# SamvitJ/Accel

Hardware: AMD Instinct MI355X
Metric: frames/sec 1024x2048 Accel-18 kf=5 (higher is better)
Workload: dtype f32 (storage, accumulation and results; the launch geometries the tuner picks include the fp32 MFMA, Winograd F(2x2,3x3) and, for most layers, 'fp16x2': each fp32 operand as TWO half terms hi + lo (22-23 significant bits, operands centred in the half range by exact powers of two: weights per channel

## Files before the change

### accel_amd/csrc/accel_hip.cpp

```cpp
#include <hip/hip_runtime.h>
#include <dlfcn.h>
#include <sys/stat.h>
#include <unistd.h>

#include <algorithm>
#include <cmath>
#include <cstdarg>
#include <cstdio>
#include <cstdlib>
#include <cstring>
#include <map>
#include <memory>
#include <sstream>
#include <string>
#include <vector>

#include "../../include/accel_hip.h"
#include "kernels.h"
#include "range.h"

static thread_local std::string g_err;

static int fail(int code, const char* fmt, ...)
{
// ... 474 lines not shown
        c.yH = op.b.H; c.yW = op.b.W;
        if (op.b.H > 2 * op.a.H || op.b.H < 2 * op.a.H - 1 || op.b.W > 2 * op.a.W || op.b.W < 2 * op.a.W - 1)
            return fail(ACCEL_ERR_PLAN, "deconv2x %s: output must be 2x the input (or one row / column less)", op.name.c_str());
    } else {
        int wkh = kh, wkw = kw;
        if (cols) kv_pair(kv, "wk", wkh, wkw, 3, 3);
        if (w->shape[0] != cout || w->shape[1] != cin || w->shape[2] != wkh || w->shape[3] != wkw)
            return fail(ACCEL_ERR_PARAM, "shape inconsistent for %s: need (%d,%d,%d,%d) got (%ld,%ld,%ld,%ld)",
                        wname.c_str(), cout, cin, wkh, wkw, (long)w->shape[0], (long)w->shape[1], (long)w->shape[2], (long)w->shape[3]);
        const int Kreal = wkh * wkw * cin_pad;
        c.K_pad = roundup(Kreal, 32);
        pack_conv_w(*w, cin_pad, rows, c.K_pad, packed);
        if (cols) { c.kh = c.kw = 1; c.Cin = Kreal; }
        else { c.kh = kh; c.kw = kw; c.Cin = cin_pad; }
        c.sh = sh; c.sw = sw; c.ph = ph; c.pw = pw; c.dh = dh; c.dw = dw;
        c.Ho = op.b.H; c.Wo = op.b.W;
        c.yH = op.b.H; c.yW = op.b.W;
        const int eh = (op.a.H + 2 * c.ph - c.dh * (c.kh - 1) - 1) / c.sh + 1;
        const int ew = (op.a.W + 2 * c.pw - c.dw * (c.kw - 1) - 1) / c.sw + 1;
        if (eh != op.b.H || ew != op.b.W)
            return fail(ACCEL_ERR_PLAN, "conv %s: output %dx%d does not match geometry %dx%d", op.name.c_str(), op.b.H, op.b.W, eh, ew);
        if (c.Cin > op.a.Cs) return fail(ACCEL_ERR_PLAN, "conv %s: input view narrower than Cin", op.name.c_str());
    }
    packed.resize(packed.size() + 256, 0.f);
    const char* env_dt = getenv("ACCEL_CONV_DTYPE");
    const int dflt = (p->f16 == 2 || (env_dt && !strcmp(env_dt, "bf16x3"))) ? 2 : (p->f16 || (env_dt && !strcmp(env_dt, "f16"))) ? 1 : 0;
    const int want_f16 = (int)kv_int(kv, "f16", dflt);
    c.f16 = (want_f16 && c.Cin % (want_f16 == 2 ? 4 : 8) == 0 && cout_store > 4) ? want_f16 : 0;
    void* dw_ = nullptr;
    if (c.f16 == 2) {
        std::vector<uint16_t> pb;
        pack_bf16x3(packed, c.deconv2x ? 4 : 1, rows, c.K_pad, pb, c.w_plane);
        if ((rc = dev_upload(p, pb.data(), pb.size() * sizeof(uint16_t), &dw_))) return rc;
    } else if (c.f16) {
        std::vector<_Float16> ph(packed.size());
        for (size_t i = 0; i < packed.size(); ++i) ph[i] = (_Float16)packed[i];
        if ((rc = dev_upload(p, ph.data(), ph.size() * sizeof(_Float16), &dw_))) return rc;
        if (!withheld("b3r")) {
            const int classes = c.deconv2x ? 4 : 1, steps = c.K_pad / 32;
            c.w_plane = (size_t)classes * rows * c.K_pad + 2 * (size_t)rows * 32;
            std::vector<_Float16> pr(c.w_plane, (_Float16)0.f);
            for (int cl = 0; cl < classes; ++cl)
                for (int n = 0; n < rows; ++n)
                    for (int k = 0; k < c.K_pad; ++k)
                        pr[((((size_t)cl * steps + k / 32) * 2 + ((k >> 4) & 1)) * rows + n) * 16 + (k & 15)] = ph[((size_t)cl * rows + n) * c.K_pad + k];
            void* d4 = nullptr;
            if ((rc = dev_upload(p, pr.data(), pr.size() * sizeof(_Float16), &d4))) return rc;
            c.wb3r = d4;
        }
    } else if ((rc = dev_upload(p, packed.data(), packed.size() * sizeof(float), &dw_))) return rc;
    c.w = static_cast<const float*>(dw_);
    {
        const int ft = (int)kv_int(kv, "tile", -1);
        const bool forced = (ft >= CONV_TILE_B3 && ft < CONV_TILE_B3D + CONV_TILE_B3D_N) || (ft >= 90 && ft <= 96);
        if (!c.f16 && c.Cin % 4 == 0 && cout_store > 4 && (!withheld("split") || forced)) {
            std::vector<uint16_t> pb;
            pack_bf16x3(packed, c.deconv2x ? 4 : 1, rows, c.K_pad, pb, c.w_plane);
            void* d3 = nullptr;
            if ((rc = dev_upload(p, pb.data(), pb.size() * sizeof(uint16_t), &d3))) return rc;
            c.wb3 = d3;
            const bool forced_r = (ft >= CONV_TILE_B3R && ft < CONV_TILE_B3D + CONV_TILE_B3D_N) || (ft >= 90 && ft <= 96);
            if (!withheld("b3r") || forced_r) {
                pack_bf16x3r(packed, c.deconv2x ? 4 : 1, rows, c.K_pad, pb, c.w_plane);
                void* d4 = nullptr;
                if ((rc = dev_upload(p, pb.data(), pb.size() * sizeof(uint16_t), &d4))) return rc;
                c.wb3r = d4;
            }
        } else if (forced && !(c.f16 == 1 && c.wb3r && ft >= CONV_TILE_B3R && ft < CONV_TILE_B3D + CONV_TILE_B3D_N)) {
            return fail(ACCEL_ERR_ARG, "conv %s: the bf16x3 kernel takes layers with more than "
                                       "4 output channels only", op.name.c_str());
        }
    }

    std::vector<float> scale(rows, 0.f), shift(rows, 0.f);
    for (int i = 0; i < cout; ++i) scale[i] = 1.f;
    if (kv_has(kv, "bn")) {
        std::vector<float> s, b;
        if ((rc = bn_fold(m, kv_str(kv, "bn"), (float)kv_f(kv, "eps", 1e-5), (int)kv_int(kv, "fixg", 0), cout, s, b))) return rc;
        for (int i = 0; i < cout; ++i) { scale[i] = s[i]; shift[i] = b[i]; }
    }
    if (kv_has(kv, "bias")) {
        const HostParam* bias = get_param(m, kv_str(kv, "bias"));
        if (!bias) return fail(ACCEL_ERR_PARAM, "%s not initialized", kv_str(kv, "bias").c_str());
        if ((int)bias->numel() != cout) return fail(ACCEL_ERR_PARAM, "shape inconsistent for %s", kv_str(kv, "bias").c_str());
        for (int i = 0; i < cout; ++i) shift[i] += bias->data[i] * scale[i];
    }
    if (kv_has(kv, "mul")) {
        const float mul = (float)kv_f(kv, "mul", 1.0);
        for (int i = 0; i < cout; ++i) { scale[i] *= mul; shift[i] *= mul; }
    }
    void *ds = nullptr, *db = nullptr;
    if ((rc = dev_upload(p, scale.data(), rows * sizeof(float), &ds)) ||
        (rc = dev_upload(p, shift.data(), rows * sizeof(float), &db))) return rc;
    c.scale = static_cast<const float*>(ds);
    c.shift = static_cast<const float*>(db);
    {
        const char* sp = getenv("ACCEL_SPLIT");
        const bool h2 = sp ? !strcmp(sp, "h2") : p->split == 1;
        if (c.wb3r && !c.f16 && h2) {
            std::vector<uint16_t> ph;
            std::vector<int> q;
            pack_h2r(packed, c.deconv2x ? 4 : 1, rows, c.K_pad, ph, c.w_plane, q);
            void *dh = nullptr, *dsh = nullptr;
            if ((rc = dev_upload(p, ph.data(), ph.size() * sizeof(uint16_t), &dh))) return rc;
            std::vector<float> sh(rows);
            for (int i = 0; i < rows; ++i) sh[i] = std::ldexp(scale[i], -q[i]);
            if ((rc = dev_upload(p, sh.data(), rows * sizeof(float), &dsh))) return rc;
            c.wh2r = dh;
            c.scale_h2 = static_cast<const float*>(dsh);
            ++p->n_h2;
        }
    }
    if (op.c.set) {
        std::vector<float> s2(rows, 0.f), b2(rows, 0.f), s, b;
// ... 95 lines not shown
        } else if (c.force_tile == CONV_TILE_WINO || c.force_tile == CONV_TILE_WINO_B3 || c.force_tile == CONV_TILE_WINO_B3U || c.force_tile == CONV_TILE_WINO_B3S) {
            return fail(ACCEL_ERR_ARG, "conv %s: the Winograd kernel takes 3x3 / stride 1 / dilation 1 / pad 1 layers with even output "
                                       "size and channels in multiples of 8 only", op.name.c_str());
        }
    }
    {
        const bool want = !withheld("stem") || c.force_tile == CONV_TILE_STEM || c.force_tile == CONV_TILE_STEM_B3;
        c.Cout_store = cout_store;
        c.res = op.d.set ? op.d.ptr : nullptr;
        if (want && !cols && cin == 3 && cout == 64 && conv_stem_eligible(c)) {
            std::vector<float> ws((size_t)conv_stem_pack_floats(), 0.f);
            conv_stem_pack(w->data.data(), cout, ws.data());
            void* dsw = nullptr;
            if ((rc = dev_upload(p, ws.data(), ws.size() * sizeof(float), &dsw))) return rc;
            c.wstem = static_cast<const float*>(dsw);
            if ((!withheld("split") && !withheld("stem_split")) || c.force_tile == CONV_TILE_STEM_B3) {
                std::vector<unsigned short> wb;
                conv_stem_b3_pack(w->data.data(), cout, wb);
                void* dsb = nullptr;
                if ((rc = dev_upload(p, wb.data(), wb.size() * sizeof(unsigned short), &dsb))) return rc;
                c.wstemb = dsb;
                if (c.wh2r) {
                    std::vector<int> q;
                    conv_stem_b3_pack_h2(w->data.data(), cout, wb, q);
                    void *dh = nullptr, *dsh = nullptr;
                    if ((rc = dev_upload(p, wb.data(), wb.size() * sizeof(unsigned short), &dh))) return rc;
                    std::vector<float> sh(rows, 0.f);
                    for (int i = 0; i < rows && i < 64; ++i) sh[i] = std::ldexp(scale[i], -q[i]);
                    if ((rc = dev_upload(p, sh.data(), rows * sizeof(float), &dsh))) return rc;
                    c.wstemh = dh;
                    c.scale_h2s = static_cast<const float*>(dsh);
                }
            }
        } else if (c.force_tile == CONV_TILE_STEM || c.force_tile == CONV_TILE_STEM_B3) {
            return fail(ACCEL_ERR_ARG, "conv %s: the stem kernel takes 7x7 / stride 2 / pad 3 layers on 3-channel images with 64 "
                                       "output channels only", op.name.c_str());
        }
    }
    {
        const bool want = !withheld("ws1x1") || c.force_tile == CONV_TILE_WS;
        c.y2 = op.c.set ? op.c.ptr : nullptr;
        if (want && !cols && cin == cin_pad && conv_ws_eligible(c)) {
            std::vector<float> ww(conv_ws_pack_floats(cin, cout_store), 0.f);
            conv_ws_pack(w->data.data(), cout, cin, cout_store, ww.data());
            void* dw = nullptr;
            if ((rc = dev_upload(p, ww.data(), ww.size() * sizeof(float), &dw))) return rc;
            c.wws = static_cast<const float*>(dw);
            c.wws_bytes = (unsigned)(ww.size() * sizeof(float));
        } else if (c.force_tile == CONV_TILE_WS) {
            return fail(ACCEL_ERR_ARG, "conv %s: the weight-stationary kernel takes 1x1 / stride 1 layers from 64 to a multiple of 256 "
                                       "or from 128 to a multiple of 128 channels (ReLU or no activation, one output) only", op.name.c_str());
        }
    }
    c.narrow = (cout_store == 4 && !c.deconv2x && !op.c.set && c.force_tile < 0 && kv_int(kv, "narrow", 1)) ? 1 : 0;
    c.no_split = (int)kv_int(kv, "nosplit", 0);
    c.split_target = (int)kv_int(kv, "split_target", 0);
    const size_t ws = conv_plan_split(c);
    if (ws > p->ws_bytes) p->ws_bytes = ws;
    return 0;
}

static int upload_param(accel_plan* p, const std::string& name, size_t expect, const float** out)
{
    const HostParam* h = get_param(p->m, name);
    if (!h) return fail(ACCEL_ERR_PARAM, "%s not initialized", name.c_str());
    if (expect && h->numel() != expect) return fail(ACCEL_ERR_PARAM, "shape inconsistent for %s: %zu elements, expected %zu", name.c_str(), h->numel(), expect);
    void* d = nullptr;
    int rc = dev_upload(p, h->data.data(), h->numel() * sizeof(float), &d);
    if (rc) return rc;
    *out = static_cast<const float*>(d);
    return 0;
}

static int input_slot(accel_plan* p, const BufRef& r, const float* const** out)
{
    *out = nullptr;
    if (r.space == "A" || r.off != 0) return 0;
    DevBuf& b = p->m->pbufs[r.space];
    ++b.prep_readers;
    if (!b.slot) {
        void* d = nullptr;
        HIP_TRY(hipMalloc(&d, sizeof(void*)));
        b.slot = static_cast<const void**>(d);
        HIP_TRY(hipMemcpy(d, &b.ptr, sizeof(void*), hipMemcpyHostToDevice));
    }
    *out = reinterpret_cast<const float* const*>(b.slot);
    return 0;
}

static int scores_buffer(accel_plan* p, Op& op, const ScoreTailParams& q)
{
    const int zCs = roundup(q.ncls, 4);
    const size_t zbytes = (size_t)op.a.N * q.Hs * q.Ws * zCs * sizeof(float);
    DevBuf& zb = p->m->pbufs["scores"];
    if (!zb.ptr) {
        HIP_TRY(hipMalloc(&zb.ptr, zbytes));
        zb.bytes = zbytes;
        HIP_TRY(hipMemsetAsync(zb.ptr, 0, zbytes, p->m->ctx->stream));
    } else if (zb.bytes != zbytes) {
        return fail(ACCEL_ERR_PLAN, "score_tail %s: the model's `scores` buffer has %zu bytes, this plan needs %zu", op.name.c_str(), zb.bytes, zbytes);
    }
    op.tail_z = static_cast<float*>(zb.ptr);
    op.tail_lowres = q;
    op.tail_lowres.left = op.tail_z; op.tail_lowres.lCs = zCs;
    op.tail_lowres.right = nullptr; op.tail_lowres.wr = nullptr;
    op.tail_lowres.uniform_w = 1;
// ... 211 lines not shown
    const ConvParams& c = op.conv;
    hipError_t e = hipSuccess;
    if (op.measure) e = launch_range_amax(c.x, (long)op.a.N * c.H * c.W, c.Cin, c.xCs, const_cast<unsigned*>(c.xr_slot), p->m->ctx->stream);
    if (e == hipSuccess && (op.measure || op.fold)) e = launch_range_fold(const_cast<unsigned*>(c.xr_slot), p->range_flag_dev, (int)(&op - p->ops.data()), p->m->ctx->stream);
    if (e != hipSuccess) return fail(ACCEL_ERR_HIP, "range pass of conv %s failed: %s", op.name.c_str(), hipGetErrorString(e));
    return 0;
}

static int run_eager(accel_plan* p)
{
    if (p->n_slots && launch_range_clear(p->range, p->n_slots, p->m->ctx->stream) != hipSuccess)
        return fail(ACCEL_ERR_HIP, "clearing the range slots of plan '%s' failed", p->role.c_str());
    for (size_t i = 0; i < p->ops.size(); ++i) {
        Op& op = p->ops[i];
        int rc = (op.measure || op.fold) ? launch_measure(p, op) : 0;
        if (!rc) rc = launch_op(p, op);
        if (rc) return rc;
        static const char* chk = getenv("ACCEL_CHECK_FINITE");
        if (chk && chk[0] == '1' && !p->gexec && (op.kind == OP_CONV || op.kind == OP_POOL || op.kind == OP_PREP_RGB) && p->n_slots) {
            const BufRef& o = op.b;
            if (o.esize == 4 && o.ptr && p->check_scratch) {
                unsigned* scratch = p->check_scratch;
                hipStream_t st = p->m->ctx->stream;
                launch_range_clear(scratch, 1, st);
                launch_range_amax(o.ptr, (long)o.N * o.H * o.W, roundup(o.C, 4), o.Cs, scratch, st);
                launch_range_fold(scratch, nullptr, 0, st);
                unsigned bits = 0;
                hipStreamSynchronize(st);
                hipMemcpy(&bits, scratch, 4, hipMemcpyDeviceToHost);
                if (bits >= 0x7F800000u) fprintf(stderr, "[accel check] plan %s op %zu %s %s: output holds a non-finite value (largest |x| bits 0x%08x)\n", p->role.c_str(), i, op.kind_name.c_str(), op.name.c_str(), bits);
            }
        }
    }
    return 0;
}

static int range_check(accel_plan* p)
{
    if (!p->range_flag || !*p->range_flag) return 0;
    const unsigned w = *p->range_flag, i = (w & 0x7FFFFFFFu) - 1u;
    *p->range_flag = 0u;
    return fail(ACCEL_ERR_RANGE, "plan '%s': the input of conv %s was not finite in an earlier run (the largest |value| stored into it was %s; fp16x2 "
                "form of the fp32 layers: the frames of that run are not trustworthy; ACCEL_SPLIT=b3 selects the bf16x3 form, which propagates "
                "non-finite values like fp32 arithmetic)",
                p->role.c_str(), i < p->ops.size() ? p->ops[i].name.c_str() : "?", (w & 0x80000000u) ? "a NaN" : "an infinity");
}

static bool conv_has_h2_form(const ConvParams& c) { return c.wh2r || c.wubh || c.wstemh; }
static bool conv_runs_h2(const ConvParams& c)
{
    if (c.f16 || c.narrow) return false;
    const int t = c.force_tile;
    return ((t == CONV_TILE_WINO_B3 || t == CONV_TILE_WINO_B3U || t == CONV_TILE_WINO_B3S) && c.wubh) || (t == CONV_TILE_STEM_B3 && c.wstemh) ||
           (((t >= CONV_TILE_B3R && t < CONV_TILE_B3R + 6) || (t >= 90 && t <= 96)) && c.wh2r);
}

static int assign_range_slots(accel_plan* p)
{
    std::map<int, int>& slot_of = p->slot_of;
    int n = 0;
    p->in_slot.assign(p->ops.size(), -1);
    for (size_t i = 0; i < p->ops.size(); ++i) {
        Op& op = p->ops[i];
        if (op.kind != OP_CONV || !conv_has_h2_form(op.conv)) continue;
        if (op.rs_in < 0) p->in_slot[i] = n++;
        else {
            auto it = slot_of.find(op.rs_in);
            if (it == slot_of.end()) it = slot_of.insert({op.rs_in, n++}).first;
            p->in_slot[i] = it->second;
        }
    }
    p->n_slots = n;
    if (!n) return 0;
    HIP_TRY(hipMalloc((void**)&p->range, (size_t)(n + 1) * RANGE_WORDS * sizeof(unsigned)));
    p->owned.push_back(p->range);
    HIP_TRY(hipMemset(p->range, 0, (size_t)(n + 1) * RANGE_WORDS * sizeof(unsigned)));
    p->check_scratch = p->range + (size_t)n * RANGE_WORDS;
    HIP_TRY(hipHostMalloc((void**)&p->range_flag, 2 * sizeof(unsigned), hipHostMallocMapped));
    p->range_flag[0] = p->range_flag[1] = 0u;
    HIP_TRY(hipHostGetDevicePointer((void**)&p->range_flag_dev, p->range_flag, 0));
    for (size_t i = 0; i < p->ops.size(); ++i)
        if (p->in_slot[i] >= 0) p->ops[i].conv.xr_slot = p->range + (size_t)p->in_slot[i] * RANGE_WORDS;
    return 0;
}

static void resolve_range_flags(accel_plan* p, bool (*counts)(const ConvParams&))
{
    const int n = p->n_slots;
    if (!n) return;
    std::vector<char> used(n, 0);
    for (size_t i = 0; i < p->ops.size(); ++i)
        if (p->in_slot[i] >= 0 && counts(p->ops[i].conv)) used[p->in_slot[i]] = 1;
    auto addr = [&](int id) -> unsigned* {
        auto it = id < 0 ? p->slot_of.end() : p->slot_of.find(id);
        return (it == p->slot_of.end() || !used[it->second]) ? nullptr : p->range + (size_t)it->second * RANGE_WORDS;
    };
    std::vector<int> state(n, 0);
    std::vector<char> dirty(n, 0);
    auto wrote = [&](int id, bool has_epilogue) {
        auto it = id < 0 ? p->slot_of.end() : p->slot_of.find(id);
        if (it == p->slot_of.end()) return;
        int& st = state[it->second];
        st = (has_epilogue && st != 2) ? 1 : 2;
        dirty[it->second] = 1;
    };
    for (size_t i = 0; i < p->ops.size(); ++i) {
        Op& op = p->ops[i];
// ... 128 lines not shown
    const char* e = getenv("ACCEL_AUTOTUNE");
    if (e && e[0] == '0') return 0;
    hipStream_t st = p->m->ctx->stream;
    tune_cache_load();
    bool tuned_any = false;
    struct Cand { int tile, split_target, no_split; };
    std::vector<std::vector<Cand>> cands(p->ops.size());
    size_t ws_need = p->ws_bytes;
    for (size_t i = 0; i < p->ops.size(); ++i) {
        Op& op = p->ops[i];
        if (op.kind != OP_CONV || op.conv.force_tile >= 0 || op.conv.narrow) continue;
        ConvParams c = op.conv;
        std::vector<Cand>& cs = cands[i];
        if (c.x_half || c.y_half || c.res_half) {
            for (int t : {CONV_TILE_B3D, CONV_TILE_B3D + 1, CONV_TILE_B3D + 2, CONV_TILE_B3D + 3, CONV_TILE_B3D + 6, CONV_TILE_B3D + 7}) {
                if ((t == CONV_TILE_B3D || t == CONV_TILE_B3D + 1) && c.Cout_store <= 128) continue;
                if ((t != CONV_TILE_B3D + 6) && c.Cout_store <= 64) continue;
                cs.push_back({t, 0, 0});
                ConvParams q = c;
                const size_t base = conv_apply(q, t, 0, 0);
                const int ks0 = q.ksplit;
                if (conv_apply(q, t, 1024, 0) && q.ksplit != ks0) cs.push_back({t, 1024, 0});
                if (base) cs.push_back({t, 0, 1});
            }
        }
        else if (c.f16 && c.Cout_store <= 32) { cs.push_back({3, 0, 0}); cs.push_back({3, 1024, 0}); }
        else if (c.Cout_store <= 32) {
            cs.push_back({4, 0, 0}); cs.push_back({4, 1024, 0}); cs.push_back({9, 0, 0}); cs.push_back({9, 1024, 0}); cs.push_back({3, 0, 0});
            if (c.wh2r && conv_halo_eligible(c) && !withheld("halo")) cs.push_back({CONV_TILE_HALO, 0, 1});
        }
        else {
            if (c.wu && !c.f16) {
                cs.push_back({CONV_TILE_WINO, 0, 0});
                ConvParams q = c;
                const size_t base = conv_apply(q, CONV_TILE_WINO, 0, 0);
                const int ks0 = q.ksplit;
                if (conv_apply(q, CONV_TILE_WINO, 1024, 0) && q.ksplit != ks0) cs.push_back({CONV_TILE_WINO, 1024, 0});
                if (base) cs.push_back({CONV_TILE_WINO, 0, 1});
            }
            if (c.wub && !c.f16) {
                for (int wt : {CONV_TILE_WINO_B3, CONV_TILE_WINO_B3U, CONV_TILE_WINO_B3S}) {
                    cs.push_back({wt, 0, 0});
                    ConvParams q = c;
                    const size_t base = conv_apply(q, wt, 0, 0);
                    const int ks0 = q.ksplit;
                    if (conv_apply(q, wt, 1024, 0) && q.ksplit != ks0) cs.push_back({wt, 1024, 0});
                    if (base) cs.push_back({wt, 0, 1});
                }
            }
            if (c.wstem && !c.f16) cs.push_back({CONV_TILE_STEM, 0, 0});
            if (c.wstemb && !c.f16) cs.push_back({CONV_TILE_STEM_B3, 0, 0});
            if (c.wws && !c.f16) cs.push_back({CONV_TILE_WS, 0, 0});
            if (c.wh2r && !c.f16 && conv_halo_eligible(c) && !withheld("halo")) cs.push_back({CONV_TILE_HALO, 0, 1});
            const int nb3 = c.wb3 ? 5 : 0;
            static const int tiles[] = {0, 1, 2, 3, 5, 6, 7, 8, 10, 11, 12, 13, 31, 32, 33, 34, 35,
                                        CONV_TILE_B3, CONV_TILE_B3 + 1, CONV_TILE_B3 + 2, CONV_TILE_B3 + 3, CONV_TILE_B3 + 4, CONV_TILE_B3 + 5,
                                        CONV_TILE_B3R, CONV_TILE_B3R + 1, CONV_TILE_B3R + 3, CONV_TILE_B3R + 4, CONV_TILE_B3R + 5};
            const bool no_deep = withheld("deep");
            for (int t : tiles) {
                if (t >= CONV_TILE_B3 && t < CONV_TILE_B3R && !nb3) continue;
                if (t >= CONV_TILE_B3R && !c.wb3r) continue;
                if (no_deep && t >= 31 && t <= 35) continue;
                if (c.K_pad % conv_tile_bk(t)) continue;
                if (c.f16 && !(t <= 3 || t == 10 || (c.f16 == 1 && t >= CONV_TILE_B3R && c.wb3r))) continue;
                cs.push_back({t, 0, 0});
                ConvParams q = c;
                const size_t base = conv_apply(q, t, 0, 0);
                const int ks0 = q.ksplit;
                if (conv_apply(q, t, 1024, 0) && q.ksplit != ks0) cs.push_back({t, 1024, 0});
                if (base) cs.push_back({t, 0, 1});
            }
        }
        if (const char* fw = getenv("ACCEL_WB3_FORCE"); fw && c.wub && !c.f16) {
            cs.clear();
            conv_apply(op.conv, atoi(fw), 0, 0);
            ConvParams q = op.conv;
            const size_t w = conv_plan_split(q);
            if (w > ws_need) ws_need = w;
            continue;
        }
        for (const Cand& k : cs) { ConvParams q = c; size_t w = conv_apply(q, k.tile, k.split_target, k.no_split); if (w > ws_need) ws_need = w; }
    }
    if (ws_need > p->ws_bytes) {
        float* nw = nullptr;
        HIP_TRY(hipMalloc((void**)&nw, ws_need));
        poison(nw, ws_need);
        p->owned.push_back(nw);
        p->ws = nw; p->ws_bytes = ws_need;
        for (Op& op : p->ops) if (op.kind == OP_CONV) op.conv.ws = p->ws;
    }
    struct TuneScratch {
        hipEvent_t e0 = nullptr, e1 = nullptr;
        void* scrub = nullptr;
        hipStream_t st;
        ~TuneScratch()
        {
            if (e0) hipEventDestroy(e0);
            if (e1) hipEventDestroy(e1);
            if (scrub) { hipStreamSynchronize(st); hipFree(scrub); }
        }
    } ts;
    ts.st = st;
    HIP_TRY(hipEventCreate(&ts.e0)); HIP_TRY(hipEventCreate(&ts.e1));
    hipEvent_t e0 = ts.e0, e1 = ts.e1;
    int rc = 0;
    const size_t scrub_bytes = (size_t)320 << 20;
// ... 1437 lines not shown
```

### accel_amd/csrc/conv_igemm.hip

```cpp
#include <hip/hip_runtime.h>
#include <cstdlib>
#include "kernels.h"
#include "conv_common.h"

#ifdef ACCEL_CONV_TIMELINE
__device__ unsigned long long g_conv_timeline[8 * 16384];
#define CONV_TL(slot) do { if (threadIdx.x == 0 && blockIdx.y == 0 && blockIdx.z == 0 && blockIdx.x < 16384) \
        g_conv_timeline[blockIdx.x * 8 + (slot)] = __builtin_amdgcn_s_memrealtime(); } while (0)
extern "C" int accel_debug_conv_timeline(unsigned long long* out, int n)
{
    return (int)hipMemcpyFromSymbol(out, HIP_SYMBOL(g_conv_timeline), sizeof(unsigned long long) * (size_t)n);
}
#else
#define CONV_TL(slot) do { } while (0)
#endif

#include "conv_epilogue.h"

template <int BM, int BN, int WGM, int WGN, int BK, int MID, int ABL = 0, int FAST = 0>
__global__ __launch_bounds__(64 * WGM * WGN) void conv_igemm_f32_kernel(ConvParams p)
{
    constexpr int LDK = BK + 4;
    constexpr int NTHR = 64 * WGM * WGN;
    constexpr int CPR = BK / 4;
// ... 935 lines not shown
    ConvParams p = p0;
    p.MT = (p.M + BM - 1) / BM;
    p.NT = (p.Cout_store + BN - 1) / BN;
    constexpr bool WDMA = WGM * WGN == 8;
    constexpr size_t lds = WDMA ? (size_t)(3 * BM * 40 + 2 * 3 * BN * 32) * sizeof(unsigned short) : (size_t)3 * (BM + BN) * 40 * sizeof(unsigned short);
    if (hipError_t e = ensure_dynamic_lds(reinterpret_cast<const void*>(&conv_igemm_b3_kernel<BM, BN, WGM, WGN, WDMA, true>), lds); e != hipSuccess) return e;
    if (hipError_t e = ensure_dynamic_lds(reinterpret_cast<const void*>(&conv_igemm_b3_kernel<BM, BN, WGM, WGN, WDMA, false>), lds); e != hipSuccess) return e;
    dim3 grid(p.MT * p.NT, p.deconv2x ? 4 : 1, p.ksplit > 1 ? p.ksplit : 1);
    if (p.Cin % 32 == 0) hipLaunchKernelGGL((conv_igemm_b3_kernel<BM, BN, WGM, WGN, WDMA, true>), grid, dim3(64 * WGM * WGN), lds, st, p, p.w_plane);
    else hipLaunchKernelGGL((conv_igemm_b3_kernel<BM, BN, WGM, WGN, WDMA, false>), grid, dim3(64 * WGM * WGN), lds, st, p, p.w_plane);
    hipError_t e = hipGetLastError();
    if (e != hipSuccess || p.ksplit <= 1) return e;
    const long total = (long)grid.y * p.M * (p.Cout_store / 4);
    hipLaunchKernelGGL(splitk_reduce_kernel, dim3((unsigned)((total + 255) / 256)), dim3(256), 0, st, p, (int)grid.y);
    return hipGetLastError();
}

int conv_pick_tile(const ConvParams& p)
{
    if (p.force_tile >= 0) return p.force_tile;
    if (p.x_half || p.y_half || p.res_half) return p.Cout_store <= 64 ? CONV_TILE_B3D + 6 : CONV_TILE_B3D + 2;
    const long classes = p.deconv2x ? 4 : 1;
    const int cs = p.Cout_store;
    if (cs <= 32) return p.f16 ? 3 : 4;
    auto blocks = [&](int bm, int bn) {
        return classes * ((p.M + bm - 1) / bm) * (long)((cs + bn - 1) / bn);
    };
    if (cs <= 64) return blocks(128, 64) >= 512 ? 1 : 3;
    if (blocks(128, 128) < 64) return 3;
    if (cs % 128 == 0 || cs > 256) {
        if (blocks(128, 128) >= 512) return 0;
        if (blocks(128, 64) >= 512) return 1;
        if (blocks(64, 128) >= 384) return 2;
        return 3;
    }
    if (blocks(128, 64) >= 512) return 1;
    return 3;
}

hipError_t launch_splitk_reduce(const ConvParams& p, int classes, hipStream_t st)
{
    const long total = (long)classes * p.M * (p.Cout_store / 4);
    hipLaunchKernelGGL(splitk_reduce_kernel, dim3((unsigned)((total + 255) / 256)), dim3(256), 0, st, p, classes);
    return hipGetLastError();
}

int conv_tile_bk(int tile) { return tile == 13 ? 64 : tile == 15 ? 16 : 32; }

bool conv_tile_valid(int tile)
{
#ifdef ACCEL_CONV_DIAG
    if ((tile >= 20 && tile <= 30) || (tile >= 90 && tile <= 96)) return true;
#endif
    return (tile >= 0 && tile <= 19) || (tile >= 31 && tile <= 35) || tile == CONV_TILE_WINO || tile == CONV_TILE_WINO_B3 || tile == CONV_TILE_WINO_B3U || tile == CONV_TILE_WINO_B3S || tile == CONV_TILE_STEM || tile == CONV_TILE_STEM_B3 || tile == CONV_TILE_WS || tile == CONV_TILE_HALO ||
           (tile >= CONV_TILE_B3 && tile < CONV_TILE_B3 + 8) || (tile >= CONV_TILE_B3R + 3 && tile <= CONV_TILE_B3R + 5) ||
           (tile >= CONV_TILE_B3D && tile < CONV_TILE_B3D + CONV_TILE_B3D_N);
}

static void tile_dims(int tile, int& bm, int& bn)
{
    static const int BMs[20] = {128, 128, 64, 64, 128, 128, 128, 64, 64, 128, 128, 128, 64, 64, 256, 128, 128, 64, 128, 64};
    static const int BNs[20] = {128, 64, 128, 64, 32, 128, 64, 128, 64, 32, 128, 64, 128, 64, 128, 128, 128, 64, 128, 64};
    if (tile == CONV_TILE_B3 + 5) { bm = 256; bn = 128; return; }
    if (tile == CONV_TILE_B3R || (tile >= 90 && tile <= 96)) { bm = 128; bn = 128; return; }
    if (tile == CONV_TILE_B3R + 1) { bm = 128; bn = 64; return; }
    if (tile == CONV_TILE_B3R + 3 || tile == CONV_TILE_B3R + 4) { bm = 128; bn = 256; return; }
    if (tile == CONV_TILE_B3R + 5) { bm = 128; bn = 128; return; }
    if (tile == CONV_TILE_B3D || tile == CONV_TILE_B3D + 4) { bm = 256; bn = 256; return; }
    if (tile == CONV_TILE_B3D + 1 || tile == CONV_TILE_B3D + 5) { bm = 128; bn = 256; return; }
    if (tile == CONV_TILE_B3D + 2 || tile == CONV_TILE_B3D + 3) { bm = 128; bn = 128; return; }
    if (tile == CONV_TILE_B3D + 6) { bm = 128; bn = 64; return; }
    if (tile == CONV_TILE_B3D + 7) { bm = 256; bn = 128; return; }
    if (tile >= CONV_TILE_B3 && tile < CONV_TILE_B3 + 5) { static const int g[5] = {0, 1, 2, 3, 10}; tile = g[tile - CONV_TILE_B3]; }
    if (tile >= 31 && tile <= 35) { static const int g[5] = {3, 0, 2, 1, 4}; tile = g[tile - 31]; }
    if (tile >= 20) tile = (tile == 23 || (tile >= 26 && tile != 29)) ? 3 : 0;
    if (tile < 0 || tile > 19) tile = 3;
    bm = BMs[tile]; bn = BNs[tile];
}

size_t conv_plan_split(ConvParams& p)
{
    p.ksplit = 1; p.kt_per_split = 0;
    if (p.no_split || p.narrow) return 0;
    int bm, bn;
    const int tile = conv_pick_tile(p);
    if (tile == CONV_TILE_STEM || tile == CONV_TILE_STEM_B3 || tile == CONV_TILE_WS || tile == CONV_TILE_HALO) return 0;
    if (tile == CONV_TILE_WINO) {
        const long blocks = ((p.M / 4 + 63) / 64) * (long)conv_wino_rows(p.Cout_store) / 64;
        const int KT = p.Cin / 8, min_steps = 4;
        const int min_blocks = p.split_target > 0 ? p.split_target : 256;
        const int target = p.split_target > 0 ? p.split_target : 512;
        if (blocks >= min_blocks || KT < 2 * min_steps) return 0;
        int want = (int)((target + blocks - 1) / blocks);
        int ks = want < KT / min_steps ? want : KT / min_steps;
        if (ks < 2) return 0;
        p.kt_per_split = ((KT + ks - 1) / ks + 1) / 2 * 2;
        p.ksplit = (KT + p.kt_per_split - 1) / p.kt_per_split;
        if (p.ksplit < 2) { p.ksplit = 1; p.kt_per_split = 0; return 0; }
        return (size_t)p.ksplit * p.M * p.Cout_store * sizeof(float);
    }
    if (tile == CONV_TILE_WINO_B3 || tile == CONV_TILE_WINO_B3U || tile == CONV_TILE_WINO_B3S) {
        const long blocks = (tile == CONV_TILE_WINO_B3U ? conv_wino_b3u_blocks(p, nullptr) : tile == CONV_TILE_WINO_B3S ? conv_wino_b3s_blocks(p, nullptr) : (long)((p.M / 4 + 63) / 64)) * (long)conv_wino_rows(p.Cout_store) / 64;
        const int KT = p.Cin / 16, min_steps = 4;
        const int min_blocks = p.split_target > 0 ? p.split_target : 256;
        const int target = p.split_target > 0 ? p.split_target : 512;
        if (blocks >= min_blocks || KT < 2 * min_steps) return 0;
        int want = (int)((target + blocks - 1) / blocks);
        int ks = want < KT / min_steps ? want : KT / min_steps;
        if (ks < 2) return 0;
        p.kt_per_split = (KT + ks - 1) / ks;
        p.ksplit = (KT + p.kt_per_split - 1) / p.kt_per_split;
        if (p.ksplit < 2) { p.ksplit = 1; p.kt_per_split = 0; return 0; }
        return (size_t)p.ksplit * p.M * p.Cout_store * sizeof(float);
    }
    tile_dims(tile, bm, bn);
    const long classes = p.deconv2x ? 4 : 1;
    const long blocks = classes * ((p.M + bm - 1) / bm) * ((p.Cout_store + bn - 1) / bn);
    const int KT = p.K_pad / conv_tile_bk(tile);
    const int min_blocks = p.split_target > 0 ? p.split_target : 256;
    const int target = p.split_target > 0 ? p.split_target : 768;
    const int min_steps = 4;
    if (blocks >= min_blocks || KT < 2 * min_steps) return 0;
    int want = (int)((target + blocks - 1) / blocks);
    int ks = want < KT / min_steps ? want : KT / min_steps;
    if (ks < 2) return 0;
    p.kt_per_split = (KT + ks - 1) / ks;
    if (tile >= CONV_TILE_B3D && tile < CONV_TILE_B3D + CONV_TILE_B3D_N && p.f16 == 1) p.kt_per_split = (p.kt_per_split + 1) / 2 * 2;
    p.ksplit = (KT + p.kt_per_split - 1) / p.kt_per_split;
    if (p.ksplit < 2) { p.ksplit = 1; p.kt_per_split = 0; return 0; }
    return (size_t)p.ksplit * classes * p.M * p.Cout_store * sizeof(float);
}

hipError_t launch_conv_igemm(const ConvParams& p, hipStream_t st)
{
    if (p.narrow) return launch_conv_narrow(p, st);
    if (p.force_tile == CONV_TILE_WINO) return launch_conv_wino(p, st);
    if (p.force_tile == CONV_TILE_WINO_B3 || p.force_tile == CONV_TILE_WINO_B3U || p.force_tile == CONV_TILE_WINO_B3S) {
        ConvParams q = p;
        if (p.wubh && !p.f16) {
            q.wub = p.wubh;
            q.wub_bytes = p.wub_bytes / 3 * 2;
            q.scale = p.scale_h2w;
            q.xr = p.xr_slot;
            q.f16 = 3;
        }
        if (p.force_tile == CONV_TILE_WINO_B3S) return launch_conv_wino_b3s(q, st);
        return launch_conv_wino_b3(q, st, p.force_tile == CONV_TILE_WINO_B3U);
    }
    if (p.force_tile == CONV_TILE_STEM) return launch_conv_stem(p, st);
    if (p.force_tile == CONV_TILE_STEM_B3) {
        if (p.wstemh && !p.f16) {
            ConvParams q = p;
            q.wstemb = p.wstemh;
            q.scale = p.scale_h2s;
            q.xr = p.xr_slot;
            q.f16 = 3;
            return launch_conv_stem_b3(q, st);
        }
        return launch_conv_stem_b3(p, st);
    }
    if (p.force_tile == CONV_TILE_WS) return launch_conv_ws(p, st);
    if (p.force_tile == CONV_TILE_HALO) {
        if (p.f16 || !p.wh2r || p.x_half || p.y_half || p.res_half) return hipErrorInvalidValue;
        ConvParams q = p;
        q.w = static_cast<const float*>(p.wh2r);
        q.w_bytes = p.w_bytes / 2;
        q.scale = p.scale_h2;
        q.xr = p.xr_slot;
        q.f16 = 3;
        return launch_conv_halo(q, st);
    }
    const int b3d_tile = (p.force_tile < 0 && (p.x_half || p.y_half || p.res_half)) ? conv_pick_tile(p) : p.force_tile;
    if (b3d_tile >= CONV_TILE_B3D && b3d_tile < CONV_TILE_B3D + CONV_TILE_B3D_N) {
        if (!p.wb3r || p.f16 != 1) return hipErrorInvalidValue;
        ConvParams q = p;
        q.w = static_cast<const float*>(p.wb3r);
        return launch_conv_b3d(q, b3d_tile, st);
    }
    if (p.x_half || p.y_half || p.res_half) return hipErrorInvalidValue;
    if (p.force_tile >= CONV_TILE_B3R && p.force_tile < CONV_TILE_B3R + 6 && p.f16 == 1) {
        if (!p.wb3r) return hipErrorInvalidValue;
        ConvParams q = p;
        q.w = static_cast<const float*>(p.wb3r);
        return launch_conv_b3r(q, p.force_tile, st);
    }
    if (((p.force_tile >= CONV_TILE_B3R && p.force_tile < CONV_TILE_B3R + 6) || (p.force_tile >= 90 && p.force_tile <= 96)) && !p.f16 && p.wh2r) {
        ConvParams q = p;
        q.w = static_cast<const float*>(p.wh2r);
        q.w_bytes = p.w_bytes / 2;
        q.scale = p.scale_h2;
        q.xr = p.xr_slot;
        q.f16 = 3;
        return launch_conv_b3r(q, p.force_tile, st);
    }
    if (((p.force_tile >= CONV_TILE_B3R && p.force_tile < CONV_TILE_B3R + 6) || (p.force_tile >= 90 && p.force_tile <= 96)) && !p.f16) {
        if (!p.wb3r) return hipErrorInvalidValue;
        ConvParams q = p;
        q.w = static_cast<const float*>(p.wb3r);
        q.w_bytes = p.w_bytes / 2;
        q.f16 = 2;
        return launch_conv_b3r(q, p.force_tile, st);
    }
    if (p.force_tile >= CONV_TILE_B3 && p.force_tile < CONV_TILE_B3 + 6 && !p.f16) {
        if (!p.wb3) return hipErrorInvalidValue;
        ConvParams q = p;
        q.w = static_cast<const float*>(p.wb3);
        q.w_bytes = p.w_bytes / 2;
        q.f16 = 2;
        switch (p.force_tile - CONV_TILE_B3) {
            case 0: return launch_b3<128, 128, 2, 2>(q, st);
            case 1: return launch_b3<128, 64, 2, 2>(q, st);
            case 2: return launch_b3<64, 128, 2, 2>(q, st);
            case 3: return launch_b3<64, 64, 2, 2>(q, st);
            case 5: return launch_b3<256, 128, 4, 2>(q, st);
// ... 71 lines not shown
```

### accel_amd/csrc/kernels.h

```cpp
#pragma once
#include <vector>
#include <hip/hip_runtime.h>
#include <stddef.h>

struct ConvParams {
    const float* x;
    const float* w;
    float* y;
    float* y2;
    const float* res;
    const float* scale; const float* shift;
    const float* scale2; const float* shift2;
    int H, W;
    int Cin;
    int xCs;
    int Ho, Wo;
    int kh, kw, sh, sw, ph, pw, dh, dw;
    int K_pad;
    int Cout_store;
    int Cout;
    int yCs, y2Cs, resCs;
    int M;
    int act;
    float slope;
// ... 34 lines not shown
    const float* scale_h2w;
    const unsigned* xr;
    const unsigned* xr_slot;
    unsigned* yr;
    unsigned* y2r;
    int x_half, y_half, res_half;
};

hipError_t launch_conv_igemm(const ConvParams& p, hipStream_t st);
int conv_pick_tile(const ConvParams& p);
int conv_tile_bk(int tile);
bool conv_tile_valid(int tile);
#define CONV_TILE_WINO 40
#define CONV_TILE_WINO_B3S 43
#define CONV_TILE_WINO_B3U 42
#define CONV_TILE_WINO_B3 41
bool conv_wino_eligible(const ConvParams& p);
int conv_wino_rows(int cout_store);
void conv_wino_pack(const float* w, int Cout, int Cin, int cin_pad, int rows, float* out);
hipError_t launch_conv_wino(const ConvParams& p, hipStream_t st);
bool conv_wino_b3_eligible(const ConvParams& p);
void conv_wino_b3_pack(const float* w, int Cout, int Cin, int rows, std::vector<unsigned short>& out);
void conv_wino_b3_pack_h2(const float* w, int Cout, int Cin, int rows, std::vector<unsigned short>& out, std::vector<int>& qexp);
hipError_t launch_conv_wino_b3(const ConvParams& p, hipStream_t st, bool union_loader = false);
long conv_wino_b3u_blocks(const ConvParams& p, int* bhs);
long conv_wino_b3s_blocks(const ConvParams& p, int* bhs);
hipError_t launch_conv_wino_b3s(const ConvParams& p, hipStream_t st);
hipError_t launch_splitk_reduce(const ConvParams& p, int classes, hipStream_t st);
#define CONV_TILE_STEM 50
#define CONV_TILE_STEM_B3 51
bool conv_stem_b3_eligible(const ConvParams& p);
void conv_stem_b3_pack(const float* w, int Cout, std::vector<unsigned short>& out);
void conv_stem_b3_pack_h2(const float* w, int Cout, std::vector<unsigned short>& out, std::vector<int>& qexp);
hipError_t launch_conv_stem_b3(const ConvParams& p, hipStream_t st);
bool conv_stem_eligible(const ConvParams& p);
void conv_stem_pack(const float* w, int Cout, float* out);
int conv_stem_pack_floats();
hipError_t launch_conv_stem(const ConvParams& p, hipStream_t st);
#define CONV_TILE_HALO 78
bool conv_halo_eligible(const ConvParams& p);
hipError_t launch_conv_halo(const ConvParams& p, hipStream_t st);
#define CONV_TILE_B3 70
#define CONV_TILE_B3R 76
hipError_t launch_conv_b3r(const ConvParams& p, int tile, hipStream_t st);
#define CONV_TILE_B3D 82
#define CONV_TILE_B3D_N 8
bool conv_b3d_eligible(const ConvParams& p);
hipError_t launch_conv_b3d(const ConvParams& p, int tile, hipStream_t st);
#define CONV_TILE_WS 60
bool conv_ws_eligible(const ConvParams& p);
size_t conv_ws_pack_floats(int Cin, int cout_store);
void conv_ws_pack(const float* w, int Cout, int Cin, int cout_store, float* out);
hipError_t launch_conv_ws(const ConvParams& p, hipStream_t st);
size_t conv_plan_split(ConvParams& p);

hipError_t launch_prep_rgb(const float* src, float* dst, int H, int W,
                           const float* scale3, const float* shift3, int N, hipStream_t st, const float* const* slot = nullptr, unsigned* yr = nullptr);
hipError_t launch_prep_flow(const float* cur, const float* prev, float* dst, int H, int W,
                            int N, hipStream_t st, const float* const* cur_slot = nullptr, const float* const* prev_slot = nullptr, unsigned* yr = nullptr);
hipError_t launch_set_slot(const void** slot, const void* value, hipStream_t st);
hipError_t launch_frames_u8(const unsigned char* src, int n, int h, int w, size_t pitch, const double* means_bgr, int out_h, int out_w, double step,
                            int H, int W, float* dst, hipStream_t st);
hipError_t launch_labels_source(const unsigned char* labels, int n, int H, int W, int out_h, int out_w, int h, int w, unsigned char* dst, size_t dst_pitch,
                                hipStream_t st);
hipError_t launch_labels_hist(const unsigned char* labels, int n, int H, int W, int out_h, int out_w, const unsigned char* gt, int h, int w, size_t gt_pitch,
                              int ncls, unsigned long long* hist, hipStream_t st);
hipError_t launch_labels_colour(const unsigned char* labels, int n, int H, int W, int out_h, int out_w, int h, int w, const unsigned char* palette_rgb,
                                int rgb_order, const unsigned char* frame, size_t frame_pitch, int alpha, unsigned char* dst, size_t dst_pitch, hipStream_t st);

struct PoolParams {
    const float* x; float* y;
    int C4;
    int xCs, yCs;
    int H, W, Ho, Wo;
    int kh, kw, sh, sw, ph, pw;
    int is_max;
    const float* scale; const float* shift;
    int relu;
    int N;
    size_t x_img, y_img;
    unsigned* yr;
};
hipError_t launch_pool(const PoolParams& p, hipStream_t st);

hipError_t launch_flow_warp(const float* feat, int fCs, const float* flow, int flCs,
                            float* out, int oCs, int C, int H, int W,
                            float* out2, int o2Cs, const float* bias, int N, hipStream_t st, unsigned* yr = nullptr, unsigned* y2r = nullptr);

struct DcnColsParams {
    const float* x; const float* off; float* col;
    int C, xCs, offCs, colCs;
    int H, W, Ho, Wo;
    int kh, kw, sh, sw, ph, pw, dh, dw;
    int dg;
    int N;
    int col_half;
    unsigned* yr;
};
hipError_t launch_dcn_cols(const DcnColsParams& p, hipStream_t st);

struct ScoreTailParams {
    const float* left;  int lCs;
    const float* right; int rCs;
    const float* wl; const float* wr;
    const float* cw; const float* cb;
    float* logits;
// ... 21 lines not shown
```

Baseline: 642.3.

## Add activation-stationary fp16x2 1x1 conv kernel as autotuner candidate

Adds a new 1x1 convolution kernel for stride 1 or 2 layers with up to 512 input channels. Each block loads its 64-row activation tile once into LDS, already split into hi/lo halves, then loops over all output-channel chunks while streaming the fp16x2 weights through a register ring buffer. This avoids re-reading and re-splitting activations for every output tile. The tuner adds it as one more candidate, so it only runs where it is measured faster. The cost is a large dynamic LDS footprint, which may limit occupancy.

Result: no change. 642.0 (-0.0%).

```diff
diff --git a/accel_amd/csrc/accel_hip.cpp b/accel_amd/csrc/accel_hip.cpp
--- a/accel_amd/csrc/accel_hip.cpp
+++ b/accel_amd/csrc/accel_hip.cpp
@@ -550,14 +550,14 @@
     c.w = static_cast<const float*>(dw_);
     {
         const int ft = (int)kv_int(kv, "tile", -1);
-        const bool forced = (ft >= CONV_TILE_B3 && ft < CONV_TILE_B3D + CONV_TILE_B3D_N) || (ft >= 90 && ft <= 96);
+        const bool forced = (ft >= CONV_TILE_B3 && ft < CONV_TILE_B3D + CONV_TILE_B3D_N) || (ft >= 90 && ft <= 96) || ft == CONV_TILE_AS;
         if (!c.f16 && c.Cin % 4 == 0 && cout_store > 4 && (!withheld("split") || forced)) {
             std::vector<uint16_t> pb;
             pack_bf16x3(packed, c.deconv2x ? 4 : 1, rows, c.K_pad, pb, c.w_plane);
             void* d3 = nullptr;
             if ((rc = dev_upload(p, pb.data(), pb.size() * sizeof(uint16_t), &d3))) return rc;
             c.wb3 = d3;
-            const bool forced_r = (ft >= CONV_TILE_B3R && ft < CONV_TILE_B3D + CONV_TILE_B3D_N) || (ft >= 90 && ft <= 96);
+            const bool forced_r = (ft >= CONV_TILE_B3R && ft < CONV_TILE_B3D + CONV_TILE_B3D_N) || (ft >= 90 && ft <= 96) || ft == CONV_TILE_AS;
             if (!withheld("b3r") || forced_r) {
                 pack_bf16x3r(packed, c.deconv2x ? 4 : 1, rows, c.K_pad, pb, c.w_plane);
                 void* d4 = nullptr;
@@ -759,6 +759,9 @@
                                        "or from 128 to a multiple of 128 channels (ReLU or no activation, one output) only", op.name.c_str());
         }
     }
+    if (c.force_tile == CONV_TILE_AS && (!c.wh2r || c.f16 || !conv_as_eligible(c)))
+        return fail(ACCEL_ERR_ARG, "conv %s: the activation-stationary kernel takes 1x1 / pad 0 / stride 1 or 2 layers in the fp16x2 form with "
+                                   "input channels in multiples of 32 up to 512 only", op.name.c_str());
     c.narrow = (cout_store == 4 && !c.deconv2x && !op.c.set && c.force_tile < 0 && kv_int(kv, "narrow", 1)) ? 1 : 0;
     c.no_split = (int)kv_int(kv, "nosplit", 0);
     c.split_target = (int)kv_int(kv, "split_target", 0);
@@ -1076,7 +1079,7 @@
     if (c.f16 || c.narrow) return false;
     const int t = c.force_tile;
     return ((t == CONV_TILE_WINO_B3 || t == CONV_TILE_WINO_B3U || t == CONV_TILE_WINO_B3S) && c.wubh) || (t == CONV_TILE_STEM_B3 && c.wstemh) ||
-           (((t >= CONV_TILE_B3R && t < CONV_TILE_B3R + 6) || (t >= 90 && t <= 96)) && c.wh2r);
+           (((t >= CONV_TILE_B3R && t < CONV_TILE_B3R + 6) || (t >= 90 && t <= 96) || t == CONV_TILE_AS) && c.wh2r);
 }
 
 static int assign_range_slots(accel_plan* p)
@@ -1311,6 +1314,7 @@
             if (c.wstemb && !c.f16) cs.push_back({CONV_TILE_STEM_B3, 0, 0});
             if (c.wws && !c.f16) cs.push_back({CONV_TILE_WS, 0, 0});
             if (c.wh2r && !c.f16 && conv_halo_eligible(c) && !withheld("halo")) cs.push_back({CONV_TILE_HALO, 0, 1});
+            if (c.wh2r && !c.f16 && conv_as_eligible(c) && !withheld("expand1x1")) cs.push_back({CONV_TILE_AS, 0, 0});
             const int nb3 = c.wb3 ? 5 : 0;
             static const int tiles[] = {0, 1, 2, 3, 5, 6, 7, 8, 10, 11, 12, 13, 31, 32, 33, 34, 35,
                                         CONV_TILE_B3, CONV_TILE_B3 + 1, CONV_TILE_B3 + 2, CONV_TILE_B3 + 3, CONV_TILE_B3 + 4, CONV_TILE_B3 + 5,
diff --git a/accel_amd/csrc/conv_1x1as.hip b/accel_amd/csrc/conv_1x1as.hip
--- /dev/null
+++ b/accel_amd/csrc/conv_1x1as.hip
@@ -0,0 +1,152 @@
+#include <hip/hip_runtime.h>
+#include "kernels.h"
+#include "conv_common.h"
+#include "conv_epilogue.h"
+
+typedef _Float16 f16x8a __attribute__((ext_vector_type(8)));
+
+#define AS_MAX_CIN 512
+
+template <int MI, int D, int OCC>
+__global__ __launch_bounds__(256, OCC) void conv_1x1as_kernel(ConvParams p, size_t wplane, int rowsB)
+{
+    constexpr int BM = 32 * MI, WGN = 4, NI = 1, BN = 32 * WGN * NI, NTHR = 64 * WGN;
+    extern __shared__ __attribute__((aligned(16))) unsigned short smem_as[];
+    const int LDA = p.Cin + 8;
+
+    const int tid = threadIdx.x, lane = tid & 63, wn = tid >> 6;
+    const int nblk = p.MT, bid = blockIdx.x;
+    const int q8 = nblk >> 3, r8 = nblk & 7, xcd = bid & 7;
+    const int mt = (xcd < r8 ? xcd * (q8 + 1) : r8 * (q8 + 1) + (xcd - r8) * q8) + (bid >> 3);
+    const int m0 = mt * BM;
+    const int HoWo = p.Ho * p.Wo;
+    const RangeScale rs = range_prologue(p.xr);
+    const float xs = rs.s;
+
+    {
+        const __amdgpu_buffer_rsrc_t xr = make_rsrc(p.x, p.x_bytes);
+        const int gpr = p.Cin >> 3, total = BM * gpr;
+        const float inv_gpr = 1.0f / (float)gpr;
+        const bool unit = p.sh == 1 && p.sw == 1;
+        constexpr int GB = 4;
+        for (int base = 0; base < total; base += NTHR * GB) {
+            f32x4 lo4[GB], hi4[GB];
+            int dst[GB];
+#pragma unroll
+            for (int u = 0; u < GB; ++u) {
+                const int idx = base + u * NTHR + tid;
+                int row, g;
+                divmod_small(idx, gpr, inv_gpr, row, g);
+                const int m = m0 + row;
+                const bool ok = idx < total && m < p.M;
+                int pix = m;
+                if (!unit) {
+                    const int mm = ok ? m : 0;
+                    const int n = mm / HoWo, rem = mm - n * HoWo;
+                    const int oy = rem / p.Wo, ox = rem - oy * p.Wo;
+                    pix = (n * p.H + oy * p.sh) * p.W + ox * p.sw;
+                }
+                const unsigned off = ok ? ((unsigned)pix * (unsigned)p.xCs + (unsigned)(g * 8)) * 4u : OOB;
+                lo4[u] = buf_load4(xr, off);
+                hi4[u] = buf_load4(xr, ok ? off + 16u : OOB);
+                dst[u] = idx < total ? row * LDA + g * 8 : -1;
+            }
+#pragma unroll
+            for (int u = 0; u < GB; ++u) {
+                f16x8a h, l;
+#pragma unroll
+                for (int e = 0; e < 8; ++e) {
+                    const float v = e < 4 ? lo4[u][e] : hi4[u][e - 4];
+                    h[e] = (_Float16)(v * xs);
+                    l[e] = (_Float16)__builtin_fmaf(v, xs, -(float)h[e]);
+                }
+                if (dst[u] >= 0) {
+                    *reinterpret_cast<i32x4*>(smem_as + dst[u]) = __builtin_bit_cast(i32x4, h);
+                    *reinterpret_cast<i32x4*>(smem_as + BM * LDA + dst[u]) = __builtin_bit_cast(i32x4, l);
+                }
+            }
+        }
+    }
+
+    const int frow = lane & 31, half = lane >> 5;
+    const __amdgpu_buffer_rsrc_t wall = make_rsrc(p.w, (unsigned)(2 * wplane) + (unsigned)((size_t)rowsB * p.K_pad * 2) + (unsigned)(rowsB * 128));
+    const unsigned b_voff = (unsigned)((wn * 32 + frow) * 32 + half * 16);
+    const unsigned hstep = (unsigned)rowsB * 32u, plane_b = (unsigned)(2 * wplane);
+    const int nh = p.K_pad >> 4, nchunk = (p.Cout_store + BN - 1) / BN;
+    i32x4 fb[D][2];
+    auto load_b = [&](int c, int hs, int buf) {
+#pragma unroll
+        for (int pl = 0; pl < 2; ++pl)
+            fb[buf][pl] = __builtin_amdgcn_raw_buffer_load_b128(wall, b_voff + (unsigned)(c * BN * 32), (unsigned)pl * plane_b + (unsigned)hs * hstep, 0);
+    };
+#pragma unroll
+    for (int u = 0; u < D; ++u) load_b(0, u, u);
+    __syncthreads();
+
+    i32x4 fa[2][MI][2];
+    auto read_fa = [&](int hs, int set) {
+        const unsigned short* a = smem_as + frow * LDA + half * 8 + hs * 16;
+#pragma unroll
+        for (int pl = 0; pl < 2; ++pl)
+#pragma unroll
+            for (int i = 0; i < MI; ++i) fa[set][i][pl] = *reinterpret_cast<const i32x4*>(a + (pl * BM + i * 32) * LDA);
+    };
+
+    for (int c = 0; c < nchunk; ++c) {
+        f32x16 acc[MI][NI];
+#pragma unroll
+        for (int i = 0; i < MI; ++i)
+#pragma unroll
+            for (int e = 0; e < 16; ++e) acc[i][0][e] = 0.f;
+        read_fa(0, 0);
+        for (int hs = 0; hs < nh; hs += D) {
+#pragma unroll
+            for (int u = 0; u < D; ++u) {
+                const int set = u & 1;
+                if (u + 1 < D) read_fa(hs + u + 1, set ^ 1);
+                else if (hs + D < nh) read_fa(hs + D, set ^ 1);
+                const f16x8a b0 = __builtin_bit_cast(f16x8a, fb[u][0]), b1 = __builtin_bit_cast(f16x8a, fb[u][1]);
+#pragma unroll
+                for (int i = 0; i < MI; ++i) {
+                    const f16x8a a0 = __builtin_bit_cast(f16x8a, fa[set][i][0]), a1 = __builtin_bit_cast(f16x8a, fa[set][i][1]);
+                    f32x16 t = acc[i][0];
+                    t = __builtin_amdgcn_mfma_f32_32x32x16_f16(a1, b0, t, 0, 0, 0);
+                    t = __builtin_amdgcn_mfma_f32_32x32x16_f16(a0, b1, t, 0, 0, 0);
+                    acc[i][0] = __builtin_amdgcn_mfma_f32_32x32x16_f16(a0, b0, t, 0, 0, 0);
+                }
+                const bool wrap = hs + u + D >= nh;
+                load_b(wrap ? c + 1 : c, wrap ? hs + u + D - nh : hs + u + D, u);
+            }
+        }
+        int m0c = m0;
+        asm volatile("" : "+s"(m0c));
+        conv_epilogue<MI, NI, WGN>(p, acc, m0c, c * BN, 0, wn, lane, 0, 0, HoWo, rs.inv);
+    }
+}
+
+bool conv_as_eligible(const ConvParams& p)
+{
+    return p.kh == 1 && p.kw == 1 && p.ph == 0 && p.pw == 0 && (p.sh == 1 || p.sh == 2) && (p.sw == 1 || p.sw == 2) && !p.deconv2x &&
+           p.Cin % 32 == 0 && p.K_pad == p.Cin && p.Cin <= AS_MAX_CIN && !p.x_half && !p.y_half && !p.res_half;
+}
+
+template <int MI, int D, int OCC>
+static hipError_t launch_as(const ConvParams& p, hipStream_t st)
+{
+    const size_t lds = (size_t)2 * (32 * MI) * (p.Cin + 8) * sizeof(unsigned short);
+    if (hipError_t e = ensure_dynamic_lds(reinterpret_cast<const void*>(&conv_1x1as_kernel<MI, D, OCC>), (size_t)2 * (32 * MI) * (AS_MAX_CIN + 8) * sizeof(unsigned short)); e != hipSuccess) return e;
+    const int rowsB = (int)(p.w_bytes / ((unsigned)p.K_pad * 2u));
+    hipLaunchKernelGGL((conv_1x1as_kernel<MI, D, OCC>), dim3(p.MT), dim3(256), lds, st, p, p.w_plane, rowsB);
+    return hipGetLastError();
+}
+
+hipError_t launch_conv_as(const ConvParams& p0, hipStream_t st)
+{
+    ConvParams p = p0;
+    if (!conv_as_eligible(p) || p.f16 != 3 || p.narrow) return hipErrorInvalidValue;
+    p.ksplit = 1; p.kt_per_split = 0;
+    p.MT = (p.M + 63) / 64;
+    p.NT = 1;
+    if (p.Cin % 64) return launch_as<2, 2, 2>(p, st);
+    return launch_as<2, 4, 2>(p, st);
+}
diff --git a/accel_amd/csrc/conv_igemm.hip b/accel_amd/csrc/conv_igemm.hip
--- a/accel_amd/csrc/conv_igemm.hip
+++ b/accel_amd/csrc/conv_igemm.hip
@@ -1011,7 +1011,7 @@
 #ifdef ACCEL_CONV_DIAG
     if ((tile >= 20 && tile <= 30) || (tile >= 90 && tile <= 96)) return true;
 #endif
-    return (tile >= 0 && tile <= 19) || (tile >= 31 && tile <= 35) || tile == CONV_TILE_WINO || tile == CONV_TILE_WINO_B3 || tile == CONV_TILE_WINO_B3U || tile == CONV_TILE_WINO_B3S || tile == CONV_TILE_STEM || tile == CONV_TILE_STEM_B3 || tile == CONV_TILE_WS || tile == CONV_TILE_HALO ||
+    return (tile >= 0 && tile <= 19) || (tile >= 31 && tile <= 35) || tile == CONV_TILE_WINO || tile == CONV_TILE_WINO_B3 || tile == CONV_TILE_WINO_B3U || tile == CONV_TILE_WINO_B3S || tile == CONV_TILE_STEM || tile == CONV_TILE_STEM_B3 || tile == CONV_TILE_WS || tile == CONV_TILE_AS || tile == CONV_TILE_HALO ||
            (tile >= CONV_TILE_B3 && tile < CONV_TILE_B3 + 8) || (tile >= CONV_TILE_B3R + 3 && tile <= CONV_TILE_B3R + 5) ||
            (tile >= CONV_TILE_B3D && tile < CONV_TILE_B3D + CONV_TILE_B3D_N);
 }
@@ -1023,6 +1023,7 @@
     if (tile == CONV_TILE_B3 + 5) { bm = 256; bn = 128; return; }
     if (tile == CONV_TILE_B3R || (tile >= 90 && tile <= 96)) { bm = 128; bn = 128; return; }
     if (tile == CONV_TILE_B3R + 1) { bm = 128; bn = 64; return; }
+    if (tile == CONV_TILE_AS) { bm = 64; bn = 128; return; }
     if (tile == CONV_TILE_B3R + 3 || tile == CONV_TILE_B3R + 4) { bm = 128; bn = 256; return; }
     if (tile == CONV_TILE_B3R + 5) { bm = 128; bn = 128; return; }
     if (tile == CONV_TILE_B3D || tile == CONV_TILE_B3D + 4) { bm = 256; bn = 256; return; }
@@ -1043,7 +1044,7 @@
     if (p.no_split || p.narrow) return 0;
     int bm, bn;
     const int tile = conv_pick_tile(p);
-    if (tile == CONV_TILE_STEM || tile == CONV_TILE_STEM_B3 || tile == CONV_TILE_WS || tile == CONV_TILE_HALO) return 0;
+    if (tile == CONV_TILE_STEM || tile == CONV_TILE_STEM_B3 || tile == CONV_TILE_WS || tile == CONV_TILE_AS || tile == CONV_TILE_HALO) return 0;
     if (tile == CONV_TILE_WINO) {
         const long blocks = ((p.M / 4 + 63) / 64) * (long)conv_wino_rows(p.Cout_store) / 64;
         const int KT = p.Cin / 8, min_steps = 4;
@@ -1119,6 +1120,16 @@
         return launch_conv_stem_b3(p, st);
     }
     if (p.force_tile == CONV_TILE_WS) return launch_conv_ws(p, st);
+    if (p.force_tile == CONV_TILE_AS) {
+        if (p.f16 || !p.wh2r || p.x_half || p.y_half || p.res_half) return hipErrorInvalidValue;
+        ConvParams q = p;
+        q.w = static_cast<const float*>(p.wh2r);
+        q.w_bytes = p.w_bytes / 2;
+        q.scale = p.scale_h2;
+        q.xr = p.xr_slot;
+        q.f16 = 3;
+        return launch_conv_as(q, st);
+    }
     if (p.force_tile == CONV_TILE_HALO) {
         if (p.f16 || !p.wh2r || p.x_half || p.y_half || p.res_half) return hipErrorInvalidValue;
         ConvParams q = p;
diff --git a/accel_amd/csrc/kernels.h b/accel_amd/csrc/kernels.h
--- a/accel_amd/csrc/kernels.h
+++ b/accel_amd/csrc/kernels.h
@@ -110,6 +110,9 @@
 size_t conv_ws_pack_floats(int Cin, int cout_store);
 void conv_ws_pack(const float* w, int Cout, int Cin, int cout_store, float* out);
 hipError_t launch_conv_ws(const ConvParams& p, hipStream_t st);
+#define CONV_TILE_AS 61
+bool conv_as_eligible(const ConvParams& p);
+hipError_t launch_conv_as(const ConvParams& p, hipStream_t st);
 size_t conv_plan_split(ConvParams& p);
 
 hipError_t launch_prep_rgb(const float* src, float* dst, int H, int W,
```
